# ersanjay16/Assignment--2-Group7-distributed-K-means

Measured on AMD Instinct MI355X. Metric: Lloyd iters/sec + points/sec, N=100M d=64 k=256, 1–8 GPUs; % of roofline, higher is better.
Workload: dtype f32; 1 GPU; c3: N=100000000 d=64 k=256; N=100000000, d=64, k=256, compute_sse=False, parallelism=dp1 (rows sharded, one RCCL all-reduce of k*(d+1) f64 per step)

## Files before the change

assignment--2-group7-distributed-k-means_amd/csrc/km_internal.h:

```cpp
#pragma once
#include <hip/hip_ext.h>
#include <hip/hip_runtime.h>
#include <stdint.h>

#include "../../include/kmeans_amd.h"

namespace km {

struct LaunchTiming {
  hipEvent_t start = nullptr, stop = nullptr;
};
extern thread_local LaunchTiming g_timing;
#define KM_TIMED_LAUNCH(KERNEL, GRID, BLOCK, LDS, STREAM, ...)                                               \
  do {                                                                                                     \
    if (::km::g_timing.start) {                                                                            \
      hipExtLaunchKernelGGL(KERNEL, GRID, BLOCK, LDS, STREAM, ::km::g_timing.start, ::km::g_timing.stop, 0, \
                            __VA_ARGS__);                                                                  \
      ::km::g_timing = ::km::LaunchTiming{};                                                               \
    } else {                                                                                               \
      hipLaunchKernelGGL(KERNEL, GRID, BLOCK, LDS, STREAM, __VA_ARGS__);                                    \
    }                                                                                                      \
  } while (0)

struct QEntry {
// ... 55 lines not shown
  int kp;
  uint32_t* qout = nullptr;
  int rev = 0;
};
hipError_t launch_assign_small(const float* X, const Geometry& g, const float* C32, const double* C64,
                               const float* cmax, int32_t* labels, double* stats, int fuse_stats, int want_sse,
                               int n_cu, const int* gate, hipStream_t s, const SmallTail& tail);
bool small_path_ok(const Geometry& g);
hipError_t launch_assign_mfma(const float* X, const Geometry& g, const _Float16* Chi, const _Float16* Clo,
                              const float* cn2s, const float* cmax, const float* xabs, const float* cabs,
                              int32_t* labels, QEntry* queue, uint32_t* qcount, int n_cu, QLayout* ql,
                              const int* gate, hipStream_t s, uint32_t* cand = nullptr, uint32_t* cand_ctr = nullptr,
                              uint32_t cand_cap = 0, int one = 0,
                              const float* C32 = nullptr, uint2* chg = nullptr, uint32_t* chg_cnt = nullptr);
int cand_rec_words();
size_t queue_capacity(int64_t n, int n_cu);
size_t qcount_words(int n_cu);
bool mfma_path_ok(const Geometry& g);
hipError_t launch_resolve(const float* X, const Geometry& g, const double* C64, const double* C64T,
                          const QEntry* queue, const uint32_t* qcount, const QLayout& ql, int32_t* labels,
                          double* stats, int n_cu, const int* gate, hipStream_t s, double* sse = nullptr,
                          const uint32_t* cand = nullptr, uint32_t cand_cap = 0, int delta = 0,
                          const float* sse_c32 = nullptr, uint2* chg = nullptr, const uint32_t* chg_cnt = nullptr,
                          const float* C32 = nullptr, const float* cmax = nullptr);
bool fused_path_ok(const Geometry& g);
#ifdef KM_DIAG
#endif
int diag_env(const char* name, int dflt);
enum { KM_SCREEN_X3 = 0, KM_SCREEN_X3_REFINE = 1, KM_SCREEN_FAST1 = 2, KM_SCREEN_FAST2 = 3 };
bool fast_path_ok(const Geometry& g);
hipError_t launch_fused(const float* X, const float* xnorm, const Geometry& g, const _Float16* Chi,
                        const _Float16* Clo, uint4* ChiF, uint4* CloF, const float* cn2s, const float* bnd,
                        const float* xabs, const float* cabs, int32_t* labels, QEntry* queue, uint32_t* qcount,
                        double* stats, int with_stats, int mode, int n_cu, QLayout* ql, const int* gate,
                        hipStream_t s, const float* C32, const float* cmax, float* bal, const double* C64P,
                        double* sse);
hipError_t launch_bound_consts(const float* cmax, const float* xabs, const float* cabs, const Geometry& g, float* bnd,
                               const int* gate, hipStream_t s);
bool fused16_ok(const Geometry& g);
hipError_t launch_row_norm(const float* X, const Geometry& g, float* xnorm, hipStream_t s);
bool stats_needs_sort(const Geometry& g, int extra);
void stats_ranges(const Geometry& g, int* fr_out, int* kr_out, int extra);
size_t sorted_stats_words(int64_t n, int k);
hipError_t launch_stats(const float* X, const Geometry& g, const int32_t* labels, const double* w, double* stats,
                        int n_cu, const int* gate, hipStream_t s, const double* C64, int c64s, const float* C32);
hipError_t launch_stats_sorted(const float* X, const Geometry& g, const int32_t* labels, const double* w,
                               double* stats, uint32_t* scratch, const double* C64P, int n_cu, const int* gate,
// ... 14 lines not shown
hipError_t launch_repair_pick(int* gate, const int64_t* counts, const Geometry& g, int64_t total,
                              double neg_log_delta, uint64_t seed, int32_t* empty, int32_t* pcounts, int64_t* picks,
                              int64_t* samples, int cp, const int64_t* sizes, const int64_t* bases, int nparts,
                              const float* X, int64_t row0, DevStatus* st, double* rows, int32_t* pending,
                              hipStream_t s);
hipError_t launch_repair_apply(int* gate, const Geometry& g, const int32_t* empty, const double* C_old,
                               double* C_new, DevStatus* st, double tol, const double* rows, const int32_t* pending,
                               hipStream_t s);
hipError_t launch_bernoulli(const uint64_t* seeds, const int64_t* sizes, const int64_t* bases, int nparts,
                            double fraction, int64_t* out, int cp, int32_t* counts, hipStream_t s);
bool s1_ok(const Geometry& g);
size_t s1_table_entries(const Geometry& g);
hipError_t launch_s1_color(const float* C32, const Geometry& g, int32_t* perm, const int* gate, hipStream_t s);
hipError_t launch_s1_prep(const double* C64, const float* C32, const Geometry& g, const int32_t* perm,
                          const float* cmax, const float* xabs, const float* cabs, float* cft, float* cn2o,
                          uint4* img, float* cst, const int* gate, hipStream_t s);
struct S1GateBufs;
hipError_t launch_s1(const float* X, const float* xnorm, const Geometry& g, const uint4* img, const float* cn2o,
                     const float* cft, const int32_t* perm, const float* cst, int32_t* labels,
                     QEntry* queue, uint32_t* qcount, uint2* chg, uint32_t* chg_cnt, int delta, int n_cu,
                     QLayout* ql, const int* gate, hipStream_t s, int rev = 0, double* sse = nullptr,
                     const S1GateBufs* gt = nullptr, int gdense = 0);
struct S1GateBufs {
  float* marg;
  uint2* wl;
  uint32_t* wl_cnt;
  double* cref;
  double* acc;
  float* accud;
};
bool s1_gate_ok(const Geometry& g);
hipError_t launch_s1_gate(const Geometry& g, const double* C64, const int32_t* labels, const S1GateBufs& b, int init,
                          const int32_t* init_dev, int n_cu, const int* gate, hipStream_t s);
size_t s1_chg_entries(const Geometry& g, int n_cu);
size_t s1_wave_slots(int n_cu);
bool s1_delta_ok(const Geometry& g, int n_cu);
hipError_t launch_s1_delta(const float* X, const Geometry& g, const uint2* chg, const uint32_t* chg_cnt,
                           double* stats, int n_cu, const int* gate, hipStream_t s, const uint32_t* qcount = nullptr);
hipError_t launch_chg_delta(const float* X, const Geometry& g, const uint2* chg, const uint32_t* chg_cnt, int nw,
                            uint32_t seg, double* stats, int n_cu, const int* gate, hipStream_t s,
                            const uint32_t* qcount = nullptr);
hipError_t launch_s1_apply(double* stats, double* full, int64_t len, int mode, const int* gate, hipStream_t s);
hipError_t launch_gen_blobs(float* X, const Geometry& g, int64_t row_offset, int32_t n_centers, float box,
                            float stddev, uint64_t seed, hipStream_t s);

__host__ __device__ inline uint64_t splitmix64(uint64_t z) {
  z += 0x9E3779B97F4A7C15ull;
// ... 18 lines not shown
```

assignment--2-group7-distributed-k-means_amd/csrc/km_kernels.hip:

```cpp
#include "km_exact.h"
#include "km_internal.h"

#include <float.h>
#include <algorithm>
#include <stdio.h>
#include <stdlib.h>

#ifndef KM_NARROW_WAVES
#define KM_NARROW_WAVES 16
#endif
#ifndef KM_WIDE_WAVES
#define KM_WIDE_WAVES 12
#endif
#ifndef KM_RERANK_PCT
#define KM_RERANK_PCT 100
#endif

namespace km {

thread_local LaunchTiming g_timing;

typedef float f32x16 __attribute__((ext_vector_type(16)));
typedef float f32x4 __attribute__((ext_vector_type(4)));

// ... 2836 lines not shown
      pre[b0 + i] = run;
      run += qcount[2 * (b0 + i) + which];
    }
  if (t == nt - 1) {
    uint32_t tot = 0;
    for (uint32_t i = 0; i < nt / 64; ++i) tot += wsum[i];
    pre[nseg] = tot;
  }
  __syncthreads();
}

__device__ __forceinline__ uint32_t find_segment(const uint32_t* __restrict__ pre, uint32_t nseg, uint32_t g) {
  uint32_t lo = 0, hi = nseg;
  while (hi - lo > 1) {
    const uint32_t mid = (lo + hi) >> 1;
    if (pre[mid] <= g)
      lo = mid;
    else
      hi = mid;
  }
  return lo;
}

template <bool WIDE, bool PF = false>
__global__ __launch_bounds__(WIDE ? 512 : 1024) void k_rerank2(const float* __restrict__ X, int dp, int d, int k,
                                                  const double* __restrict__ C64, const QEntry* __restrict__ queue,
                                                  const uint32_t* __restrict__ qcount, QLayout ql,
                                                  int32_t* __restrict__ labels, double* __restrict__ stats,
                                                  int tab_kp, double* __restrict__ sse, const int* __restrict__ gate,
                                                  const uint32_t* __restrict__ cand, uint32_t cand_cap, int delta,
                                                  const float* __restrict__ sse_c32, uint2* __restrict__ chg,
                                                  const uint32_t* __restrict__ chg_cnt,
                                                  const float* __restrict__ C32, const float* __restrict__ cmax) {
  if (*gate) return;
  extern __shared__ __attribute__((aligned(16))) char smem[];
  const float cmv = PF ? *cmax : 0.0f;
  double* tab = reinterpret_cast<double*>(smem);
  uint32_t* pre = reinterpret_cast<uint32_t*>(smem + (stats && tab_kp ? (size_t)(d + 1) * tab_kp * 8 : 0));
  uint32_t* pre1 = pre + ql.nwaves + 1;
  if (stats && tab_kp)
    for (int i = threadIdx.x; i < (d + 1) * tab_kp; i += blockDim.x) tab[i] = 0.0;
  block_prefix(qcount, 0, ql.nwaves, pre);
  if (stats && !delta) block_prefix(qcount, 1, ql.nwaves, pre1);
  const uint32_t total = pre[ql.nwaves];
  const int u = threadIdx.x & 7;
  const uint32_t ng = (gridDim.x * blockDim.x) >> 3;
  double ss_acc = 0.0;
  for (uint32_t g = (blockIdx.x * blockDim.x + threadIdx.x) >> 3; g < total + ((ng - total % ng) % ng);
       g += ng) {
    const bool have = g < total;
    QEntry q{0, 0, 0, 0};
    size_t cpos = 0;
    if (have) {
      const uint32_t sg = find_segment(pre, ql.nwaves, g);
      q = queue[(size_t)sg * ql.seg + (g - pre[sg])];
      if (delta) cpos = (size_t)sg * ql.seg + chg_cnt[sg] + (g - pre[sg]);
// ... 91 lines not shown
      mnorm = ua ? va : mnorm;
      bi = ua ? a : bi;
      const bool ub = bb != a && np_better(vb, mnorm, true);
      mnorm = ub ? vb : mnorm;
      bi = ub ? bb : bi;
    }
    lab = bi < 0 ? 0 : bi;
    if (!have) continue;
    double rsq_bad = 0.0;
    if (!ok && u == 0) {
      double best = 0.0;
      for (int j = 0; j < k; ++j) {
        const double* __restrict__ c = C64 + (size_t)j * d;
        const double v = np_norm_d<WIDE ? 5 : 2>([&](int f) { return np_sq(c[f], x[f]); }, d);
        const bool u = np_better(v, best, j > 0);
        best = u ? v : best;
        lab = u ? j : lab;
      }
      rsq_bad = best;
    }
    if (!ok) lab = __shfl(lab, (int)(threadIdx.x & 63) & ~7);
    const int old = delta ? (int)min((uint32_t)labels[q.row], (uint32_t)(k - 1)) : -1;
    if (u == 0) labels[q.row] = lab;
    if (sse && sse_c32) {
      double r = 0.0;
      for (int f = u; f < d; f += 8) {
        const double e = (double)x[f] - (double)sse_c32[(size_t)lab * dp + f];
        r = fma(e, e, r);
      }
      ss_acc += r;
    } else if (sse && u == 0) {
      const double mn = ok ? mnorm : rsq_bad;
      ss_acc += mn * mn;
    }
    if (delta) {
      if (u == 0) chg[cpos] = make_uint2(q.row, ((uint32_t)old << 16) | (uint32_t)lab);
    } else if (stats) {
      for (int f = u; f < d; f += 8) {
        if (tab_kp)
          atomicAdd(tab + (size_t)f * tab_kp + lab, (double)x[f]);
        else
          atomicAdd(stats + (size_t)lab * (d + 1) + f, (double)x[f]);
      }
      if (u == 0) {
        if (tab_kp)
          atomicAdd(tab + (size_t)d * tab_kp + lab, 1.0);
// ... 19 lines not shown
      if (u == 0) {
        if (tab_kp)
          atomicAdd(tab + (size_t)d * tab_kp + lab, 1.0);
        else
          atomicAdd(stats + (size_t)lab * (d + 1) + d, 1.0);
      }
    }
  }
  if (stats && tab_kp) {
    __syncthreads();
    for (int i = threadIdx.x; i < (d + 1) * tab_kp; i += blockDim.x) {
      const int j = i / (d + 1);
      const int f = i - j * (d + 1);
      const double v = tab[(size_t)f * tab_kp + j];
      if (v != 0.0 && j < k) atomicAdd(stats + (size_t)j * (d + 1) + f, v);
    }
  }
  if (sse) {
    ss_acc = wave_sum(ss_acc);
    if ((threadIdx.x & 63) == 0 && ss_acc != 0.0) atomicAdd(sse, ss_acc);
  }
}

template <int G, bool WIDE, bool PF = false>
__global__ __launch_bounds__(512) void k_fullscan(const float* __restrict__ X, int dp, int d, int k,
                                                   const double* __restrict__ C64T, const QEntry* __restrict__ queue,
                                                   const uint32_t* __restrict__ qcount, QLayout ql,
                                                   int32_t* __restrict__ labels, int ch,
                                                   double* __restrict__ stats, int use_chain, int pair_chain,
                                                   double* __restrict__ sse, const int* __restrict__ gate, int delta,
                                                   const float* __restrict__ sse_c32, uint2* __restrict__ chg,
                                                   const uint32_t* __restrict__ chg_cnt,
                                                   const float* __restrict__ C32, const float* __restrict__ cmax,
                                                   const double* __restrict__ C64r) {
  if (*gate) return;
  extern __shared__ __attribute__((aligned(16))) char smem[];
  double* sCT = reinterpret_cast<double*>(smem);
  float* xs_all = reinterpret_cast<float*>(smem + (size_t)d * ch * 8);
  uint32_t* pre = reinterpret_cast<uint32_t*>(smem + (size_t)d * ch * 8 + (size_t)8 * G * d * 4);
  uint32_t* kept_all = pre + ((ql.nwaves + 1u + 3u) & ~3u);
  const float cmv = PF ? *cmax : 0.0f;
  block_prefix(qcount, 1, ql.nwaves, pre);
  const uint32_t total = pre[ql.nwaves];
  const int lane = threadIdx.x & 63;
  const int wave = threadIdx.x >> 6;
  float* xs = xs_all + (size_t)wave * G * d;
  const uint32_t per_batch = 8u * G;
  double ss_acc = 0.0;
  for (uint32_t b0 = blockIdx.x * per_batch; b0 < total; b0 += gridDim.x * per_batch) {
    uint32_t rows[G];
    bool have[G];
    int chain[G];
    QEntry qe[G];
    size_t cpos[G];
#pragma unroll
    for (int g = 0; g < G; ++g) {
      const uint32_t e = b0 + (uint32_t)(wave * G + g);
// ... 23 lines not shown
#pragma unroll
      for (int g = 0; g < G; ++g)
        for (int f = 256 + lane; f < d; f += 64) xs[g * d + f] = X[(size_t)rows[g] * dp + f];
    auto finish = [&](int g, double bv, int bi) {
#pragma unroll
      for (int o = 32; o >= 1; o >>= 1) {
        const double ob = __shfl_xor(bv, o);
        const int oj = __shfl_xor(bi, o);
        bool take = false;
        if (oj >= 0) {
          if (bi < 0) {
            take = true;
          } else {
            const bool on = ob != ob, mn = bv != bv;
            take = (on && !mn) || (on == mn && (on ? oj < bi : (ob < bv || (ob == bv && oj < bi))));
          }
        }
        bv = take ? ob : bv;
        bi = take ? oj : bi;
      }
      const int lab = bi < 0 ? 0 : bi;
      const int old = delta ? (int)min((uint32_t)labels[rows[g]], (uint32_t)(k - 1)) : -1;
      if (lane == 0) labels[rows[g]] = lab;
      if (sse && sse_c32) {
        for (int f = lane; f < d; f += 64) {
          const double e = (double)xs[g * d + f] - (double)sse_c32[(size_t)lab * dp + f];
          ss_acc = fma(e, e, ss_acc);
        }
      } else if (sse && lane == 0 && bi >= 0) {
        ss_acc += bv * bv;
      }
      if (delta) {
        if (lane == 0) chg[cpos[g]] = make_uint2(rows[g], ((uint32_t)old << 16) | (uint32_t)lab);
      } else if (stats) {
        for (int f = lane; f < d; f += 64) atomicAdd(stats + (size_t)lab * (d + 1) + f, (double)xs[g * d + f]);
        if (lane == 0) atomicAdd(stats + (size_t)lab * (d + 1) + d, 1.0);
      }
    };
    if (k <= 256 && pair_chain) {
      static_assert(G % 2 == 0, "entry pairs");
#pragma unroll
      for (int p = 0; p < G; p += 2) {
        const bool a0 = have[p] && chain[p] >= 0, a1 = have[p + 1] && chain[p + 1] >= 0;
        if (!a0 && !a1) continue;
        const int e = lane >> 5;
        const int j = (e ? chain[p + 1] : chain[p]) + 8 * (lane & 31);
// ... 190 lines not shown
          const bool ua = have[g] && np_better(va, best[g], bj[g] >= 0);
          const bool ub = have[g + 1] && np_better(vb, best[g + 1], bj[g + 1] >= 0);
          best[g] = ua ? va : best[g];
          bj[g] = ua ? c0 + lane : bj[g];
          best[g + 1] = ub ? vb : best[g + 1];
          bj[g + 1] = ub ? c0 + lane : bj[g + 1];
        }
      }
    }
#pragma unroll
    for (int g = 0; g < G; ++g)
      if (have[g]) finish(g, best[g], bj[g]);
  }
  if (sse) {
    ss_acc = wave_sum(ss_acc);
    if (lane == 0 && ss_acc != 0.0) atomicAdd(sse, ss_acc);
  }
}

hipError_t launch_resolve(const float* X, const Geometry& g, const double* C64, const double* C64T,
                          const QEntry* queue, const uint32_t* qcount, const QLayout& ql, int32_t* labels,
                          double* stats, int n_cu, const int* gate, hipStream_t s, double* sse,
                          const uint32_t* cand, uint32_t cand_cap, int delta, const float* sse_c32, uint2* chg,
                          const uint32_t* chg_cnt, const float* C32, const float* cmax) {
  if (g.n == 0 || ql.nwaves == 0) return hipSuccess;
  if (delta && (!chg || !chg_cnt || g.k > 65535)) return hipErrorInvalidValue;
  if (delta) stats = nullptr;
  constexpr size_t LDS_MAX = 160 * 1024;
  const size_t pre_bytes = ((size_t)ql.nwaves + 1) * 4;
  if (pre_bytes > LDS_MAX / 4) return hipErrorInvalidValue;
  if (g.d > WIDE_MAX_DP) return hipErrorInvalidValue;
  static const int fs_g = diag_env("KM_FS_G", 0);
  const int G = fs_g == 4 ? 4 : (fs_g == 2 ? 2 : (g.k > 256 ? 4 : 2));
  const int ch = g.d <= 128 ? 64 : (g.d <= 256 ? 32 : 0);
  static const int fs_pf = diag_env("KM_FS_PF", 1);
  const bool pf = fs_pf && ch > 0 && C32 != nullptr && cmax != nullptr && g.d % 2 == 0 &&
                  (g.dp == 32 || g.dp == 64 || g.dp == 128 || g.dp == 256) && (size_t)ch * g.dp / 4 <= 4 * 512;
  const size_t fs_lds = (size_t)g.d * ch * 8 + (size_t)8 * G * g.d * 4 +
                        (pf ? (((size_t)ql.nwaves + 4) & ~(size_t)3) * 4 + (size_t)8 * G * 64 * 4 : pre_bytes);
  if (fs_lds > LDS_MAX) return hipErrorInvalidValue;
  static const int use_chain = diag_env("KM_CHAIN", 1);
  static const int pair_chain = diag_env("KM_PAIR_CHAIN", 1);
  static const int fs_wg = diag_env("KM_FS_WG", 1);
  if (ch == 0)
    hipLaunchKernelGGL((k_fullscan<2, true>), dim3(n_cu * fs_wg), dim3(512), fs_lds, s, X, g.dp, g.d, g.k, C64T,
                       queue, qcount, ql, labels, ch, (double*)nullptr, use_chain, pair_chain, sse, gate, delta, sse_c32, chg,
                       chg_cnt, C32, cmax, C64);
  else if (G == 4 && pf)
    hipLaunchKernelGGL((k_fullscan<4, false, true>), dim3(n_cu * fs_wg), dim3(512), fs_lds, s, X, g.dp, g.d, g.k,
                       C64T, queue, qcount, ql, labels, ch, (double*)nullptr, use_chain, pair_chain, sse, gate, delta,
                       sse_c32, chg, chg_cnt, C32, cmax, C64);
  else if (G == 4)
    hipLaunchKernelGGL((k_fullscan<4, false>), dim3(n_cu * fs_wg), dim3(512), fs_lds, s, X, g.dp, g.d, g.k, C64T,
                       queue, qcount, ql, labels, ch, (double*)nullptr, use_chain, pair_chain, sse, gate, delta, sse_c32, chg,
                       chg_cnt, C32, cmax, C64);
  else if (pf)
    hipLaunchKernelGGL((k_fullscan<2, false, true>), dim3(n_cu * fs_wg), dim3(512), fs_lds, s, X, g.dp, g.d, g.k,
                       C64T, queue, qcount, ql, labels, ch, (double*)nullptr, use_chain, pair_chain, sse, gate, delta,
                       sse_c32, chg, chg_cnt, C32, cmax, C64);
  else
    hipLaunchKernelGGL((k_fullscan<2, false>), dim3(n_cu * fs_wg), dim3(512), fs_lds, s, X, g.dp, g.d, g.k, C64T,
                       queue, qcount, ql, labels, ch, (double*)nullptr, use_chain, pair_chain, sse, gate, delta, sse_c32, chg,
                       chg_cnt, C32, cmax, C64);
  hipError_t e = hipGetLastError();
  if (e != hipSuccess) return e;
  const size_t tab_bytes = (size_t)(g.d + 1) * g.kp * 8;
  const size_t pres = (stats ? 2 : 1) * pre_bytes;
  const int tab_kp = (stats && !delta && tab_bytes + pres <= LDS_MAX) ? g.kp : 0;
  static const int rpct = diag_env("KM_RERANK_PCT", KM_RERANK_PCT);
  const int rwg = std::max(1, n_cu * std::max(1, rpct) / 100);
  static const int rr_pf = diag_env("KM_RR_PF", 1);
  if (g.d > 256)
    hipLaunchKernelGGL(k_rerank2<true>, dim3(rwg), dim3(512), (tab_kp ? tab_bytes : 0) + pres, s, X, g.dp, g.d,
                       g.k, C64, queue, qcount, ql, labels, stats, tab_kp, sse, gate, cand, cand_cap, delta, sse_c32, chg,
                       chg_cnt, C32, cmax);
  else if (rr_pf && g.d <= 128 && C32 && cmax)
    hipLaunchKernelGGL((k_rerank2<false, true>), dim3(rwg), dim3(1024), (tab_kp ? tab_bytes : 0) + pres, s, X, g.dp,
                       g.d, g.k, C64, queue, qcount, ql, labels, stats, tab_kp, sse, gate, cand, cand_cap, delta, sse_c32,
                       chg, chg_cnt, C32, cmax);
  else
    hipLaunchKernelGGL(k_rerank2<false>, dim3(rwg), dim3(1024), (tab_kp ? tab_bytes : 0) + pres, s, X, g.dp, g.d,
                       g.k, C64, queue, qcount, ql, labels, stats, tab_kp, sse, gate, cand, cand_cap, delta, sse_c32, chg,
                       chg_cnt, C32, cmax);
  return hipGetLastError();
}

static constexpr int STATS_LDS = 156 * 1024;

template <bool SSE, bool W>
__global__ __launch_bounds__(1024) void k_stats(const float* __restrict__ X, int64_t n, int d, int dp, int k,
                                                const int32_t* __restrict__ labels, double* __restrict__ stats,
                                                int kr, int fr, int64_t rows_per_block, const double* __restrict__ C64,
                                                const float* __restrict__ C32, double* __restrict__ sse,
                                                const int* __restrict__ gate, const double* __restrict__ w,
                                                double* __restrict__ wsum, int c64s) {
  if (*gate) return;
  if constexpr (!SSE) sse = nullptr;
  extern __shared__ __attribute__((aligned(16))) char smem[];
  double* tab = reinterpret_cast<double*>(smem);
  const int RS = fr + (W ? 2 : 1);
  const int L = fr / 4;
  const int c0 = blockIdx.y * kr;
  const int c1 = min(k, c0 + kr);
  const int f0 = blockIdx.z * fr;
  const bool counts = blockIdx.z == 0;
  const int nent = (c1 - c0) * RS;
// ... 870 lines not shown
```

assignment--2-group7-distributed-k-means_amd/csrc/km_runtime.hip:

```cpp
#include <stdlib.h>
#include <string.h>

#include <algorithm>
#include <cmath>
#include <string>
#include <utility>
#include <vector>

#include "../../include/kmeans_amd.h"
#include "km_internal.h"

namespace {
thread_local std::string g_err;

int fail(int code, const std::string& msg) {
  g_err = msg;
  return code;
}

#define KM_HIP(call)                                                                               \
  do {                                                                                             \
    hipError_t e_ = (call);                                                                        \
    if (e_ != hipSuccess)                                                                          \
      return fail(KM_ERR_HIP, std::string(#call) + ": " + hipGetErrorString(e_) + " (" +           \
// ... 522 lines not shown
  c->bounds_valid = false;
  if (!use_s1(c, with_stats)) c->gate_init_dev = nullptr;
  if (with_stats) c->last_gated = false;
  if (with_stats && !c->stats_clean) KM_HIP(hipMemsetAsync(c->stats, 0, sizeof(double) * stats_len(c), c->stream));
  if (with_stats) c->stats_clean = false;
  if (c->path == 1) {
    ProfScope ps(c, KM_K_ASSIGN, true);
    KM_HIP(km::launch_assign_small(c->X, g, c->C32, c->C64_cur, c->cmax, c->labels, c->stats, with_stats ? 1 : 0,
                                   sse ? 1 : 0, c->n_cu, c->gate, c->stream, small_tail(c)));
    c->ql = km::QLayout{0, g.n > 0 ? 1u : 0u};
    return KM_OK;
  }
  if (with_stats) {
    c->stats_pending = 1;
    c->last_delta = false;
    c->sse_corr = false;
  }
  if (use_s1(c, with_stats)) {
    double* s1_sse = sse ? sse_slot : nullptr;
    const bool gated = with_stats && !s1_sse && c->fused && g.n > 0 && km::s1_gate_ok(g);
    bool gdense = false;
    if (gated) {
      if (!c->gt.marg) {
        KM_HIP(hipMalloc(&c->gt.marg, sizeof(float) * (size_t)g.n));
        KM_HIP(hipMalloc(&c->gt.wl, sizeof(uint2) * km::s1_chg_entries(g, c->n_cu)));
        KM_HIP(hipMalloc(&c->gt.wl_cnt, sizeof(uint32_t) * km::s1_wave_slots(c->n_cu)));
        KM_HIP(hipMalloc(&c->gt.cref, sizeof(double) * (size_t)g.k * g.d));
        KM_HIP(hipMemsetAsync(c->gt.cref, 0, sizeof(double) * (size_t)g.k * g.d, c->stream));
        KM_HIP(hipMalloc(&c->gt.acc, sizeof(double) * (size_t)g.k));
        KM_HIP(hipMalloc(&c->gt.accud, sizeof(float) * 2 * (size_t)g.k));
        KM_HIP(hipMemsetAsync(c->gt.acc, 0, sizeof(double) * (size_t)g.k, c->stream));
        KM_HIP(hipMemsetAsync(c->gt.accud, 0, sizeof(float) * 2 * (size_t)g.k, c->stream));
      }
      gdense = !bounds_were_valid;
      ProfScope ps(c, KM_K_PREP);
      KM_HIP(km::launch_s1_gate(g, c->C64_cur, c->labels, c->gt, gdense ? 2 : 0, c->gate_init_dev, c->n_cu, c->gate,
                                c->stream));
    }
    c->gate_init_dev = nullptr;
    {
      ProfScope ps(c, KM_K_ASSIGN, true);
      KM_HIP(km::launch_s1(c->X, c->xnorm, g, c->s1_img, c->s1_cn2o, c->s1_cft, c->s1_perm, c->s1_cst,
                           c->labels, c->queue, c->qcount, c->chg, c->chg_cnt, with_stats ? 1 : 0, c->n_cu,
                           &c->ql, c->gate, c->stream, gated ? 0 : next_sweep(c), s1_sse,
                           gated ? &c->gt : nullptr, gdense ? 1 : 0));
    }
    if (gated) {
      c->bounds_valid = true;
      c->last_gated = true;
      c->gated_nw = c->ql.nwaves;
      c->gated_dense = gdense;
    }
    {
      ProfScope ps(c, KM_K_RESOLVE);
      KM_HIP(km::launch_resolve(c->X, g, c->C64_cur, c->C64T, c->queue, c->qcount, c->ql, c->labels, nullptr,
                                c->n_cu, c->gate, c->stream, s1_sse, nullptr, 0, with_stats ? 1 : 0,
                                s1_sse ? c->C32 : nullptr, c->chg, c->chg_cnt, c->C32, c->cmax));
    }
    if (with_stats) {
      ProfScope ps(c, KM_K_STATS);
      KM_HIP(km::launch_s1_delta(c->X, g, c->chg, c->chg_cnt, c->stats, c->n_cu, c->gate, c->stream, c->qcount));
    }
    if (with_stats) {
      c->stats_pending = 2;
      c->last_delta = true;
      c->sse_corr = s1_sse != nullptr;
    }
    return KM_OK;
  }
  if (c->fused) {
    {
      const int rc = ensure_x3(c);
      if (rc != KM_OK) return rc;
    }
    {
      ProfScope ps(c, KM_K_ASSIGN, true);
      KM_HIP(km::launch_fused(c->X, c->xnorm, g, c->Chi, c->Clo, c->ChiF, c->CloF, c->cn2s, c->bnd, c->xabs, c->cabs,
                              c->labels, c->queue, c->qcount, c->stats, with_stats ? 1 : 0,
                              (with_stats || c->screen >= km::KM_SCREEN_FAST1) ? c->screen : km::KM_SCREEN_X3_REFINE,
                              c->n_cu, &c->ql, c->gate, c->stream, c->C32, c->cmax, c->bal, c->C64P,
// ... 1157 lines not shown
```

assignment--2-group7-distributed-k-means_amd/csrc/km_s1_gate.h:

```cpp
#pragma once
#include <math.h>
#include <stdint.h>

#if defined(__HIPCC__) || defined(__CUDACC__)
#define KM_S1G_FN __host__ __device__ inline
#else
#define KM_S1G_FN inline
#endif

namespace km {

constexpr float S1G_U = 5.9604644775390625e-08f;
constexpr float S1G_TINY = 1e-30f;

KM_S1G_FN float s1g_up(float v) { return fmaf(fabsf(v), 8.0f * S1G_U, v) + S1G_TINY; }
KM_S1G_FN float s1g_dn(float v) { return fmaf(fabsf(v), -8.0f * S1G_U, v) - S1G_TINY; }

KM_S1G_FN float s1g_sqrt(float v) {
#if defined(__HIP_DEVICE_COMPILE__)
  return __builtin_amdgcn_sqrtf(v);
#else
  return sqrtf(v);
#endif
}
// ... 54 lines not shown
  const float f = (float)acc;
  const float r = fmaf(f, 0x1p-23f, f) + S1G_TINY;
  return (r <= 3.0e38f) ? r : INFINITY;
}
KM_S1G_FN float s1g_acc_dn(double acc) {
  if (!(acc <= 3.0e38)) return 0.0f;
  const float f = (float)acc;
  const float r = fmaf(f, -0x1p-23f, f) - S1G_TINY;
  return r > 0.0f ? r : 0.0f;
}
KM_S1G_FN double s1g_acc_pass(double acc, float sl, float so, float top, bool reset, float* up, float* dn) {
  const bool wild = !(top <= 3.0e38f);
  const double a = (reset || wild) ? 0.0 : s1g_acc_add(acc, sl, so);
  *up = (wild && !reset) ? INFINITY : s1g_acc_up(a);
  *dn = s1g_acc_dn(a);
  return a;
}
KM_S1G_FN float s1g_base(float marg, float acc_dn) {
  const float b = s1g_dn(marg + acc_dn);
  return (fabsf(b) <= 3.0e38f) ? b : 0.0f;
}
KM_S1G_FN bool s1g_keep(float base, float acc_up) { return base > acc_up; }

KM_S1G_FN float s1g_xnorm(float xs) {
  float v = s1g_up(xs * (1.0f + 64.0f * S1G_U));
  v = !(v < 0x1p-96f) ? v : 0x1p-96f;
  return s1g_up(s1g_up(s1g_sqrt(v)));
}

}
```

assignment--2-group7-distributed-k-means_amd/csrc/km_screen1.hip:

```cpp
#include <float.h>

#include <type_traits>

#include "km_internal.h"
#include "km_s1_gate.h"
#include "km_s1_ring.h"

namespace km {

namespace {

typedef _Float16 f16x8 __attribute__((ext_vector_type(8)));
typedef float f32x4 __attribute__((ext_vector_type(4)));
typedef float f32x2 __attribute__((ext_vector_type(2)));
typedef _Float16 f16x2 __attribute__((ext_vector_type(2)));

constexpr float U24 = 5.9604644775390625e-08f;
constexpr float U16 = 4.8828125e-04f;
#ifndef KM_S1_LMAX
#define KM_S1_LMAX 8
#endif
constexpr int S1_LMAX = KM_S1_LMAX;
#ifndef KM_S1_NBUF
#define KM_S1_NBUF 0
// ... 28 lines not shown
  const int dp = 32 * ns2, kp = 32 * nb, nt = 32 << ceil_log2_c(nb);
  return (size_t)kp * dp * 2 + (table ? (size_t)nt * (dp + 4) * 4 : 0) + (size_t)kp * 4 + (size_t)nt * 4 +
         (s1_batched(ns2) ? (size_t)s1_waves(ns2, nb) * s1_ring(ns2, nb) * (dp * 4 + 16 + 128) : 0);
}
constexpr bool s1_table_global(int ns2, int nb) { return s1_lds_bytes(ns2, nb, true) > 160 * 1024; }
#ifndef KM_S1_GATE
#define KM_S1_GATE 1
#endif
constexpr size_t s1_gate_ring_lds(int ns2, int nb) { return (size_t)s1_waves(ns2, nb) * s1_ring(ns2, nb) * 4; }
constexpr size_t s1_gate_lds(int ns2, int nb) { return s1_gate_ring_lds(ns2, nb) + (size_t)32 * nb * 4; }
constexpr bool s1_gated_with(int ns2, int nb, size_t extra) {
  return KM_S1_GATE && s1_batched(ns2) && s1_tiles(ns2) == 1 && !s1_table_global(ns2, nb) &&
         s1_lds_bytes(ns2, nb, true) + extra <= 160 * 1024;
}
constexpr bool s1_gated(int ns2, int nb) { return s1_gated_with(ns2, nb, s1_gate_lds(ns2, nb)); }
constexpr bool s1_gated_kept(int ns2, int nb) {
  return s1_gated(ns2, nb) == s1_gated_with(ns2, nb, s1_gate_ring_lds(ns2, nb));
}
static_assert(s1_gated_kept(2, 2) && s1_gated_kept(2, 4) && s1_gated_kept(2, 6) && s1_gated_kept(2, 8) &&
                  s1_gated_kept(1, 2) && s1_gated_kept(1, 4) && s1_gated_kept(1, 6) && s1_gated_kept(1, 8) &&
                  s1_gated_kept(1, 12) && s1_gated_kept(1, 16),
              "the lower totals' LDS table must not cost a geometry its gate");
static_assert(!KM_S1_GATE || !KM_S1_W12 || s1_gated(2, 8), "the c3 geometry is gated");


__device__ __forceinline__ uint32_t f2u(float v) { return __float_as_uint(v); }
__device__ __forceinline__ float u2f(uint32_t v) { return __uint_as_float(v); }

__device__ __forceinline__ float min_raw(float a, float b) {
  float r;
  asm("v_min_f32 %0, %1, %2" : "=v"(r) : "v"(a), "v"(b));
  return r;
}
__device__ __forceinline__ float min3_raw(float a, float b, float c) {
  float r;
  asm("v_min3_f32 %0, %1, %2, %3" : "=v"(r) : "v"(a), "v"(b), "v"(c));
  return r;
}

__device__ __forceinline__ float quad_min(float v) {
  auto p = __builtin_amdgcn_permlane16_swap(f2u(v), f2u(v), false, false);
  v = min_raw(u2f(p[0]), u2f(p[1]));
  p = __builtin_amdgcn_permlane32_swap(f2u(v), f2u(v), false, false);
  return min_raw(u2f(p[0]), u2f(p[1]));
}
__device__ __forceinline__ float quad_sum(float v) {
// ... 135 lines not shown
  }
}

struct S1Args {
  const float* X;
  const float* xnorm;
  int64_t n;
  int k, d;
  uint32_t seg;
  const uint4* img;
  const float* cn2o;
  const float* cft;
  const int32_t* perm;
  const float* cst;
  int32_t* labels;
  QEntry* queue;
  uint32_t* qcount;
  uint2* chg;
  uint32_t* chg_cnt;
  double* sse;
  const int* gate;
  const uint2* wl;
  const uint32_t* wl_cnt;
  float* marg;
  const float* acc_dn;
};

template <int NS2, int NB, int MODE, bool REV = false, bool SSE = false, int GATED = 0>
__global__ __launch_bounds__(s1_waves(NS2, NB) * 64, s1_waves(NS2, NB) / 4) void k_s1(S1Args A) {
  if (*A.gate) return;
  constexpr int S1_WAVES = s1_waves(NS2, NB);
  constexpr int S1_RING = s1_ring(NS2, NB);
  static_assert(S1_RING == 12 || S1_RING == 16, "ring sizes covered by s1_ring_check");
  static_assert(16 <= 2 * S1_RING && S1_TILE_ROWS == 16, "a tile may complete at most two batches");
  static_assert(!GATED || (MODE == 1 && !REV && !SSE && s1_batched(NS2)), "the gated instance: delta mode, batched");
  constexpr bool LIST = GATED == 1;
  constexpr bool MARG = GATED != 0;
  constexpr int DP = 32 * NS2;
  constexpr int FQ = 8 * NS2;
  constexpr int KP = 32 * NB;
  constexpr int MB = ceil_log2_c(NB);
  constexpr int NT = 32 << MB;
  constexpr int CS = DP + 4;
  constexpr uint32_t SLOTM = (uint32_t)NT - 1u;
  constexpr uint32_t KMASK = ~SLOTM;
  constexpr float RHO = (float)SLOTM * 1.1920928955078125e-07f * 1.0001f;
  constexpr bool BATCH = s1_batched(NS2);
// ... 228 lines not shown
      {
        const float4* hp = sRh + ((wave * S1_RING + slot) * 4 + q) * 2;
        const float4 h0 = hp[0], h1 = hp[1];
        const float hv[8] = {h0.x, h0.y, h0.z, h0.w, h1.x, h1.y, h1.z, h1.w};
        float prev = u2f(mt.w);
#pragma unroll
        for (int r = 1; r < S1_LMAX; ++r) {
          if (__ballot(act && (uint32_t)r < cnt) == 0ull) break;
          float nl = FLT_MAX;
#pragma unroll
          for (int i = 0; i < 8; ++i) nl = min_raw(nl, hv[i] > prev ? hv[i] : FLT_MAX);
          prev = quad_min(nl);
          sl[r] = (uint32_t)r < cnt ? (f2u(prev) & SLOTM) : 0u;
        }
      }
      int32_t lab1 = 0, lab2 = 0;
      uint32_t kind = 2u, ws = 0u;
      float ubw = 0.0f, lbo = 0.0f;
      decide(act, cnt, sl, xv, lab1, lab2, kind, ws, ubw, lbo);
      emit(act, mt.x, kind, lab1, lab2, (int32_t)(mt.y & 0xFFFFu));
      resid(act && kind == 0u, ws, xv);
      if constexpr (MARG) {
        if (act && q == 0)
          A.marg[mt.x] = (kind == 0u && gscale)
                             ? s1g_base(s1g_margin(fminf(lbo, sRl[wave * S1_RING + slot]), ubw), sAd[lab1])
                             : 0.0f;
      }
    } else {
      (void)nb;
    }
  };

  auto tail = [&](uint32_t tile, const Buf& B, const float (&h)[2][4], float h2m) {
    uint32_t row;
    uint32_t lold = 0u;
    if constexpr (LIST) {
      row = wpick(wg0.x, wsub);
      lold = wpick(wg0.y, wsub);
    } else {
      row = tmap(tile) * 16u + (uint32_t)c16;
    }
    const bool valid = row < n;
    float hk[2][4];
#pragma unroll
    for (int cb = 0; cb < 2; ++cb)
#pragma unroll
      for (int i = 0; i < 4; ++i) hk[cb][i] = u2f(f2u(h[cb][i]) | qbits | ((uint32_t)(16 * cb + i) << MB));

    auto mn = [](float a, float b) { return __builtin_fminf(a, b); };
// ... 67 lines not shown
    const int32_t labm = sPerm[sm];
    const bool dec1 = ok && cnt == 1u && labm >= 0;
    int32_t old = 0;
    if constexpr (LIST)
      old = (int32_t)min(lold, (uint32_t)(A.k - 1));
    else if constexpr (MODE == 1)
      old = (int32_t)min((uint32_t)B.old, (uint32_t)(A.k - 1));
#if KM_S1_ABL == 2
    emit(valid, row, dec1 || needy ? 0u : 2u, labm, 0, old);
    return;
#endif
    float lbT = 0.0f;
    if constexpr (MARG) {
      const S1GRow gr = s1g_row(s, E, xq);
      float nl = h2m;
#pragma unroll
      for (int cb = 0; cb < 2; ++cb)
#pragma unroll
        for (int i = 0; i < 4; ++i) nl = min_raw(nl, hk[cb][i] > m ? hk[cb][i] : FLT_MAX);
      const float h2 = quad_min(nl);
      lbT = s1g_lb(T, RP, gr);
      if (valid && !needy && q == 0)
        A.marg[row] =
            (dec1 && gscale) ? s1g_base(s1g_margin(s1g_lb(h2, RP, gr), s1g_ub(m, RP, gr)), sAd[labm]) : 0.0f;
    }
    if constexpr (BATCH) {
      emit(valid && !needy, row, dec1 ? 0u : 2u, labm, 0, old);
      resid(dec1, sm, B.x);
      const uint64_t mrow = __ballot(needy && q == 0);
      if (mrow) {
        const uint32_t nn = (uint32_t)__popcll(mrow);
        const uint32_t rk = (uint32_t)__popcll(mrow & ((1ull << c16) - 1ull));
        const uint32_t space = (uint32_t)S1_RING - rc;
        const uint4 meta = make_uint4(row, (uint32_t)old | (cnt << 16), sm, f2u(la));
        auto stash = [&](uint32_t slot) {
          float4* xs = reinterpret_cast<float4*>(sRx + (wave * S1_RING + slot) * DP + FQ * q);
#pragma unroll
          for (int u = 0; u < FQ / 4; ++u) xs[u] = B.x[u];
          if (q == 0) sRm[wave * S1_RING + slot] = meta;
          float4* hp = sRh + ((wave * S1_RING + slot) * 4 + q) * 2;
          hp[0] = make_float4(hk[0][0], hk[0][1], hk[0][2], hk[0][3]);
          hp[1] = make_float4(hk[1][0], hk[1][1], hk[1][2], hk[1][3]);
          if constexpr (MARG)
            if (q == 0) sRl[wave * S1_RING + slot] = lbT;
        };
        constexpr bool EARLY0 = !SSE;
        if (EARLY0 && needy && rk < space) stash(rc + rk);
// ... 282 lines not shown
      m1 = fmaxf(m1, om1);
    }
    if (lane == 0) {
      stop[0] = m1;
      stop[1] = fmaxf(m2, 0.0f);
      stop[2] = __int_as_float(a1);
    }
  }
  __syncthreads();
  {
    const float top1 = stop[0], top2 = stop[1];
    const int atop = __float_as_int(stop[2]);
    for (int j = threadIdx.x; j < k; j += blockDim.x) {
      float up, dn;
      acc[j] = s1g_acc_pass(acc[j], sv[j], j == atop ? top2 : top1, top1, reset != 0, &up, &dn);
      accud[j] = up;
      accud[k + j] = dn;
    }
  }
}

struct S1GateArgs {
  const int32_t* labels;
  const float* marg;
  int64_t n;
  int k;
  uint32_t seg;
  const float* acc_up;
  uint2* wl;
  uint32_t* wl_cnt;
  int init;
  const int32_t* init_dev;
  const int* gate;
};

constexpr int S1G_UNITS = 2;
constexpr uint32_t S1G_TRIP = 256u * S1G_UNITS;

template <int WAVES>
__global__ __launch_bounds__(WAVES * 64) void k_s1_gate(S1GateArgs A) {
  if (*A.gate) return;
  __shared__ float sUp[1024];
  for (int i = threadIdx.x; i < A.k; i += WAVES * 64) sUp[i] = A.acc_up[i];
  __syncthreads();
  const int lane = threadIdx.x & 63, wave = threadIdx.x >> 6;
  const uint32_t gw = blockIdx.x * WAVES + wave;
  const uint64_t n = (uint64_t)A.n;
  const uint64_t r0 = (uint64_t)gw * A.seg, r1 = max(r0, min(n, r0 + A.seg));
  uint2* wl = A.wl + (size_t)gw * A.seg;
  const uint64_t below = (1ull << lane) - 1ull;
  const bool init = A.init != 0 || (A.init_dev && *A.init_dev != 0);
  const uint32_t km1 = (uint32_t)(A.k - 1);
  uint32_t cnt = 0;
  struct Trip {
    int4 lab[S1G_UNITS];
    float4 bs[S1G_UNITS];
  };
  auto fetch = [&](uint64_t base, Trip& T) {
#pragma unroll
    for (int u = 0; u < S1G_UNITS; ++u) {
      const uint64_t row = base + 256u * u + 4u * (uint32_t)lane;
      T.lab[u] = *reinterpret_cast<const int4*>(A.labels + row);
      T.bs[u] = init ? make_float4(0.0f, 0.0f, 0.0f, 0.0f) : *reinterpret_cast<const float4*>(A.marg + row);
    }
  };
  auto fetch_tail = [&](uint64_t base, Trip& T) {
#pragma unroll
    for (int u = 0; u < S1G_UNITS; ++u) {
      const uint64_t row = base + 256u * u + 4u * (uint32_t)lane;
      int32_t l[4];
      float b[4];
#pragma unroll
      for (int i = 0; i < 4; ++i) {
        const bool in = row + i < r1;
        l[i] = in ? A.labels[row + i] : 0;
        b[i] = (in && !init) ? A.marg[row + i] : 0.0f;
      }
      T.lab[u] = make_int4(l[0], l[1], l[2], l[3]);
      T.bs[u] = make_float4(b[0], b[1], b[2], b[3]);
    }
  };
  auto sift = [&](uint64_t base, const Trip& T) {
#pragma unroll
    for (int u = 0; u < S1G_UNITS; ++u) {
      const uint64_t row = base + 256u * u + 4u * (uint32_t)lane;
      auto clampk = [&](int32_t v) -> uint32_t { return (uint32_t)v < km1 ? (uint32_t)v : km1; };
      const uint32_t l[4] = {clampk(T.lab[u].x), clampk(T.lab[u].y), clampk(T.lab[u].z), clampk(T.lab[u].w)};
      const float b[4] = {T.bs[u].x, T.bs[u].y, T.bs[u].z, T.bs[u].w};
      bool ls[4];
      uint32_t c = 0;
#pragma unroll
      for (int i = 0; i < 4; ++i) {
        ls[i] = row + i < r1 && (init || !s1g_keep(b[i], sUp[l[i]]));
        c += ls[i] ? 1u : 0u;
      }
      const uint64_t b0 = __ballot((c & 1u) != 0u), b1 = __ballot((c & 2u) != 0u), b2 = __ballot((c & 4u) != 0u);
      if ((b0 | b1 | b2) == 0ull) continue;
      uint32_t pos = cnt + (uint32_t)__popcll(b0 & below) + 2u * (uint32_t)__popcll(b1 & below) +
                     4u * (uint32_t)__popcll(b2 & below);
#pragma unroll
      for (int i = 0; i < 4; ++i)
        if (ls[i]) wl[pos++] = make_uint2((uint32_t)(row + i), l[i]);
      cnt += (uint32_t)__popcll(b0) + 2u * (uint32_t)__popcll(b1) + 4u * (uint32_t)__popcll(b2);
    }
  };
  const uint64_t rfull = r0 + (r1 - r0) / S1G_TRIP * S1G_TRIP;
  uint64_t base = r0;
  if (base < rfull) {
    Trip ta, tb;
    fetch(base, ta);
    tb = ta;
// ... 361 lines not shown
```

Before: 1241 Lloyd it/s.

## Pack gate margin and label into one word to halve gate-kernel reads

The S1 gate margin buffer now stores a packed 32-bit word: the margin base float with its low 9 mantissa bits replaced by the label. The screening and resolve kernels (rerank, fullscan) write this packed word, so the gate kernel reads one stream instead of both labels and margins. The gate unroll factor also rises from 2 to 4 units. In exchange, margin precision drops slightly, the resolve kernels do extra scattered writes, and labels are limited to 512.

```diff
diff --git a/assignment--2-group7-distributed-k-means_amd/csrc/km_internal.h b/assignment--2-group7-distributed-k-means_amd/csrc/km_internal.h
--- a/assignment--2-group7-distributed-k-means_amd/csrc/km_internal.h
+++ b/assignment--2-group7-distributed-k-means_amd/csrc/km_internal.h
@@ -101,7 +101,7 @@
                           double* stats, int n_cu, const int* gate, hipStream_t s, double* sse = nullptr,
                           const uint32_t* cand = nullptr, uint32_t cand_cap = 0, int delta = 0,
                           const float* sse_c32 = nullptr, uint2* chg = nullptr, const uint32_t* chg_cnt = nullptr,
-                          const float* C32 = nullptr, const float* cmax = nullptr);
+                          const float* C32 = nullptr, const float* cmax = nullptr, uint32_t* gword = nullptr);
 bool fused_path_ok(const Geometry& g);
 #ifdef KM_DIAG
 #endif
@@ -162,7 +162,7 @@
                      QLayout* ql, const int* gate, hipStream_t s, int rev = 0, double* sse = nullptr,
                      const S1GateBufs* gt = nullptr, int gdense = 0);
 struct S1GateBufs {
-  float* marg;
+  uint32_t* marg;
   uint2* wl;
   uint32_t* wl_cnt;
   double* cref;
diff --git a/assignment--2-group7-distributed-k-means_amd/csrc/km_kernels.hip b/assignment--2-group7-distributed-k-means_amd/csrc/km_kernels.hip
--- a/assignment--2-group7-distributed-k-means_amd/csrc/km_kernels.hip
+++ b/assignment--2-group7-distributed-k-means_amd/csrc/km_kernels.hip
@@ -1,5 +1,6 @@
 #include "km_exact.h"
 #include "km_internal.h"
+#include "km_s1_gate.h"
 
 #include <float.h>
 #include <algorithm>
@@ -2882,7 +2883,9 @@
   return lo;
 }
 
-template <bool WIDE, bool PF = false>
+__device__ __forceinline__ uint32_t* gate_word_of(uint32_t* p) { return p; }
+
+template <bool WIDE, bool PF = false, typename... GW>
 __global__ __launch_bounds__(WIDE ? 512 : 1024) void k_rerank2(const float* __restrict__ X, int dp, int d, int k,
                                                   const double* __restrict__ C64, const QEntry* __restrict__ queue,
                                                   const uint32_t* __restrict__ qcount, QLayout ql,
@@ -2891,7 +2894,8 @@
                                                   const uint32_t* __restrict__ cand, uint32_t cand_cap, int delta,
                                                   const float* __restrict__ sse_c32, uint2* __restrict__ chg,
                                                   const uint32_t* __restrict__ chg_cnt,
-                                                  const float* __restrict__ C32, const float* __restrict__ cmax) {
+                                                  const float* __restrict__ C32, const float* __restrict__ cmax,
+                                                  GW... gword) {
   if (*gate) return;
   extern __shared__ __attribute__((aligned(16))) char smem[];
   const float cmv = PF ? *cmax : 0.0f;
@@ -3029,6 +3033,8 @@
     if (!ok) lab = __shfl(lab, (int)(threadIdx.x & 63) & ~7);
     const int old = delta ? (int)min((uint32_t)labels[q.row], (uint32_t)(k - 1)) : -1;
     if (u == 0) labels[q.row] = lab;
+    if constexpr (sizeof...(GW) != 0)
+      if (u == 0) gate_word_of(gword...)[q.row] = s1g_pack(0.0f, (uint32_t)lab);
     if (sse && sse_c32) {
       double r = 0.0;
       for (int f = u; f < d; f += 8) {
@@ -3094,7 +3100,7 @@
   }
 }
 
-template <int G, bool WIDE, bool PF = false>
+template <int G, bool WIDE, bool PF = false, typename... GW>
 __global__ __launch_bounds__(512) void k_fullscan(const float* __restrict__ X, int dp, int d, int k,
                                                    const double* __restrict__ C64T, const QEntry* __restrict__ queue,
                                                    const uint32_t* __restrict__ qcount, QLayout ql,
@@ -3104,7 +3110,7 @@
                                                    const float* __restrict__ sse_c32, uint2* __restrict__ chg,
                                                    const uint32_t* __restrict__ chg_cnt,
                                                    const float* __restrict__ C32, const float* __restrict__ cmax,
-                                                   const double* __restrict__ C64r) {
+                                                   const double* __restrict__ C64r, GW... gword) {
   if (*gate) return;
   extern __shared__ __attribute__((aligned(16))) char smem[];
   double* sCT = reinterpret_cast<double*>(smem);
@@ -3174,6 +3180,8 @@
       const int lab = bi < 0 ? 0 : bi;
       const int old = delta ? (int)min((uint32_t)labels[rows[g]], (uint32_t)(k - 1)) : -1;
       if (lane == 0) labels[rows[g]] = lab;
+      if constexpr (sizeof...(GW) != 0)
+        if (lane == 0) gate_word_of(gword...)[rows[g]] = s1g_pack(0.0f, (uint32_t)lab);
       if (sse && sse_c32) {
         for (int f = lane; f < d; f += 64) {
           const double e = (double)xs[g * d + f] - (double)sse_c32[(size_t)lab * dp + f];
@@ -3410,9 +3418,10 @@
                           const QEntry* queue, const uint32_t* qcount, const QLayout& ql, int32_t* labels,
                           double* stats, int n_cu, const int* gate, hipStream_t s, double* sse,
                           const uint32_t* cand, uint32_t cand_cap, int delta, const float* sse_c32, uint2* chg,
-                          const uint32_t* chg_cnt, const float* C32, const float* cmax) {
+                          const uint32_t* chg_cnt, const float* C32, const float* cmax, uint32_t* gword) {
   if (g.n == 0 || ql.nwaves == 0) return hipSuccess;
   if (delta && (!chg || !chg_cnt || g.k > 65535)) return hipErrorInvalidValue;
+  if (gword && (!delta || g.kp > (1 << S1G_LBITS))) return hipErrorInvalidValue;
   if (delta) stats = nullptr;
   constexpr size_t LDS_MAX = 160 * 1024;
   const size_t pre_bytes = ((size_t)ql.nwaves + 1) * 4;
@@ -3430,26 +3439,30 @@
   static const int use_chain = diag_env("KM_CHAIN", 1);
   static const int pair_chain = diag_env("KM_PAIR_CHAIN", 1);
   static const int fs_wg = diag_env("KM_FS_WG", 1);
-  if (ch == 0)
-    hipLaunchKernelGGL((k_fullscan<2, true>), dim3(n_cu * fs_wg), dim3(512), fs_lds, s, X, g.dp, g.d, g.k, C64T,
-                       queue, qcount, ql, labels, ch, (double*)nullptr, use_chain, pair_chain, sse, gate, delta, sse_c32, chg,
-                       chg_cnt, C32, cmax, C64);
+#define KM_FS_LAUNCH(KERNEL_, ...)                                                                              \
+  hipLaunchKernelGGL(KERNEL_, dim3(n_cu * fs_wg), dim3(512), fs_lds, s, X, g.dp, g.d, g.k, C64T, queue, qcount, ql, \
+                     labels, ch, (double*)nullptr, use_chain, pair_chain, sse, gate, delta, sse_c32, chg, chg_cnt,  \
+                     C32, cmax, C64, ##__VA_ARGS__)
+  if (gword && ch == 0) return hipErrorInvalidValue;
+  if (gword && G == 4 && pf)
+    KM_FS_LAUNCH((k_fullscan<4, false, true, uint32_t*>), gword);
+  else if (gword && G == 4)
+    KM_FS_LAUNCH((k_fullscan<4, false, false, uint32_t*>), gword);
+  else if (gword && pf)
+    KM_FS_LAUNCH((k_fullscan<2, false, true, uint32_t*>), gword);
+  else if (gword)
+    KM_FS_LAUNCH((k_fullscan<2, false, false, uint32_t*>), gword);
+  else if (ch == 0)
+    KM_FS_LAUNCH((k_fullscan<2, true>));
   else if (G == 4 && pf)
-    hipLaunchKernelGGL((k_fullscan<4, false, true>), dim3(n_cu * fs_wg), dim3(512), fs_lds, s, X, g.dp, g.d, g.k,
-                       C64T, queue, qcount, ql, labels, ch, (double*)nullptr, use_chain, pair_chain, sse, gate, delta,
-                       sse_c32, chg, chg_cnt, C32, cmax, C64);
+    KM_FS_LAUNCH((k_fullscan<4, false, true>));
   else if (G == 4)
-    hipLaunchKernelGGL((k_fullscan<4, false>), dim3(n_cu * fs_wg), dim3(512), fs_lds, s, X, g.dp, g.d, g.k, C64T,
-                       queue, qcount, ql, labels, ch, (double*)nullptr, use_chain, pair_chain, sse, gate, delta, sse_c32, chg,
-                       chg_cnt, C32, cmax, C64);
+    KM_FS_LAUNCH((k_fullscan<4, false>));
   else if (pf)
-    hipLaunchKernelGGL((k_fullscan<2, false, true>), dim3(n_cu * fs_wg), dim3(512), fs_lds, s, X, g.dp, g.d, g.k,
-                       C64T, queue, qcount, ql, labels, ch, (double*)nullptr, use_chain, pair_chain, sse, gate, delta,
-                       sse_c32, chg, chg_cnt, C32, cmax, C64);
+    KM_FS_LAUNCH((k_fullscan<2, false, true>));
   else
-    hipLaunchKernelGGL((k_fullscan<2, false>), dim3(n_cu * fs_wg), dim3(512), fs_lds, s, X, g.dp, g.d, g.k, C64T,
-                       queue, qcount, ql, labels, ch, (double*)nullptr, use_chain, pair_chain, sse, gate, delta, sse_c32, chg,
-                       chg_cnt, C32, cmax, C64);
+    KM_FS_LAUNCH((k_fullscan<2, false>));
+#undef KM_FS_LAUNCH
   hipError_t e = hipGetLastError();
   if (e != hipSuccess) return e;
   const size_t tab_bytes = (size_t)(g.d + 1) * g.kp * 8;
@@ -3458,18 +3471,22 @@
   static const int rpct = diag_env("KM_RERANK_PCT", KM_RERANK_PCT);
   const int rwg = std::max(1, n_cu * std::max(1, rpct) / 100);
   static const int rr_pf = diag_env("KM_RR_PF", 1);
-  if (g.d > 256)
-    hipLaunchKernelGGL(k_rerank2<true>, dim3(rwg), dim3(512), (tab_kp ? tab_bytes : 0) + pres, s, X, g.dp, g.d,
-                       g.k, C64, queue, qcount, ql, labels, stats, tab_kp, sse, gate, cand, cand_cap, delta, sse_c32, chg,
-                       chg_cnt, C32, cmax);
+#define KM_RR_LAUNCH(KERNEL_, THREADS_, ...)                                                                     \
+  hipLaunchKernelGGL(KERNEL_, dim3(rwg), dim3(THREADS_), (tab_kp ? tab_bytes : 0) + pres, s, X, g.dp, g.d, g.k, C64, \
+                     queue, qcount, ql, labels, stats, tab_kp, sse, gate, cand, cand_cap, delta, sse_c32, chg,       \
+                     chg_cnt, C32, cmax, ##__VA_ARGS__)
+  if (gword && g.d > 128) return hipErrorInvalidValue;
+  if (gword && rr_pf && C32 && cmax)
+    KM_RR_LAUNCH((k_rerank2<false, true, uint32_t*>), 1024, gword);
+  else if (gword)
+    KM_RR_LAUNCH((k_rerank2<false, false, uint32_t*>), 1024, gword);
+  else if (g.d > 256)
+    KM_RR_LAUNCH((k_rerank2<true>), 512);
   else if (rr_pf && g.d <= 128 && C32 && cmax)
-    hipLaunchKernelGGL((k_rerank2<false, true>), dim3(rwg), dim3(1024), (tab_kp ? tab_bytes : 0) + pres, s, X, g.dp,
-                       g.d, g.k, C64, queue, qcount, ql, labels, stats, tab_kp, sse, gate, cand, cand_cap, delta, sse_c32,
-                       chg, chg_cnt, C32, cmax);
+    KM_RR_LAUNCH((k_rerank2<false, true>), 1024);
   else
-    hipLaunchKernelGGL(k_rerank2<false>, dim3(rwg), dim3(1024), (tab_kp ? tab_bytes : 0) + pres, s, X, g.dp, g.d,
-                       g.k, C64, queue, qcount, ql, labels, stats, tab_kp, sse, gate, cand, cand_cap, delta, sse_c32, chg,
-                       chg_cnt, C32, cmax);
+    KM_RR_LAUNCH((k_rerank2<false>), 1024);
+#undef KM_RR_LAUNCH
   return hipGetLastError();
 }
 
diff --git a/assignment--2-group7-distributed-k-means_amd/csrc/km_runtime.hip b/assignment--2-group7-distributed-k-means_amd/csrc/km_runtime.hip
--- a/assignment--2-group7-distributed-k-means_amd/csrc/km_runtime.hip
+++ b/assignment--2-group7-distributed-k-means_amd/csrc/km_runtime.hip
@@ -568,7 +568,7 @@
     bool gdense = false;
     if (gated) {
       if (!c->gt.marg) {
-        KM_HIP(hipMalloc(&c->gt.marg, sizeof(float) * (size_t)g.n));
+        KM_HIP(hipMalloc(&c->gt.marg, sizeof(uint32_t) * (size_t)g.n));
         KM_HIP(hipMalloc(&c->gt.wl, sizeof(uint2) * km::s1_chg_entries(g, c->n_cu)));
         KM_HIP(hipMalloc(&c->gt.wl_cnt, sizeof(uint32_t) * km::s1_wave_slots(c->n_cu)));
         KM_HIP(hipMalloc(&c->gt.cref, sizeof(double) * (size_t)g.k * g.d));
@@ -601,7 +601,8 @@
       ProfScope ps(c, KM_K_RESOLVE);
       KM_HIP(km::launch_resolve(c->X, g, c->C64_cur, c->C64T, c->queue, c->qcount, c->ql, c->labels, nullptr,
                                 c->n_cu, c->gate, c->stream, s1_sse, nullptr, 0, with_stats ? 1 : 0,
-                                s1_sse ? c->C32 : nullptr, c->chg, c->chg_cnt, c->C32, c->cmax));
+                                s1_sse ? c->C32 : nullptr, c->chg, c->chg_cnt, c->C32, c->cmax,
+                                gated ? c->gt.marg : nullptr));
     }
     if (with_stats) {
       ProfScope ps(c, KM_K_STATS);
diff --git a/assignment--2-group7-distributed-k-means_amd/csrc/km_s1_gate.h b/assignment--2-group7-distributed-k-means_amd/csrc/km_s1_gate.h
--- a/assignment--2-group7-distributed-k-means_amd/csrc/km_s1_gate.h
+++ b/assignment--2-group7-distributed-k-means_amd/csrc/km_s1_gate.h
@@ -100,6 +100,33 @@
 }
 KM_S1G_FN bool s1g_keep(float base, float acc_up) { return base > acc_up; }
 
+constexpr int S1G_LBITS = 9;
+constexpr uint32_t S1G_LMASK = (1u << S1G_LBITS) - 1u;
+
+KM_S1G_FN uint32_t s1g_bits(float v) {
+#if defined(__HIP_DEVICE_COMPILE__)
+  return __float_as_uint(v);
+#else
+  uint32_t u;
+  __builtin_memcpy(&u, &v, 4);
+  return u;
+#endif
+}
+KM_S1G_FN float s1g_float(uint32_t u) {
+#if defined(__HIP_DEVICE_COMPILE__)
+  return __uint_as_float(u);
+#else
+  float v;
+  __builtin_memcpy(&v, &u, 4);
+  return v;
+#endif
+}
+KM_S1G_FN uint32_t s1g_pack(float base, uint32_t label) {
+  return ((base > 0.0f) ? (s1g_bits(base) & ~S1G_LMASK) : 0u) | (label & S1G_LMASK);
+}
+KM_S1G_FN float s1g_word_base(uint32_t w) { return s1g_float(w & ~S1G_LMASK); }
+KM_S1G_FN uint32_t s1g_word_label(uint32_t w) { return w & S1G_LMASK; }
+
 KM_S1G_FN float s1g_xnorm(float xs) {
   float v = s1g_up(xs * (1.0f + 64.0f * S1G_U));
   v = !(v < 0x1p-96f) ? v : 0x1p-96f;
diff --git a/assignment--2-group7-distributed-k-means_amd/csrc/km_screen1.hip b/assignment--2-group7-distributed-k-means_amd/csrc/km_screen1.hip
--- a/assignment--2-group7-distributed-k-means_amd/csrc/km_screen1.hip
+++ b/assignment--2-group7-distributed-k-means_amd/csrc/km_screen1.hip
@@ -74,6 +74,13 @@
                   s1_gated_kept(1, 12) && s1_gated_kept(1, 16),
               "the lower totals' LDS table must not cost a geometry its gate");
 static_assert(!KM_S1_GATE || !KM_S1_W12 || s1_gated(2, 8), "the c3 geometry is gated");
+constexpr bool s1_gate_label_fits(int ns2, int nb) { return !s1_gated(ns2, nb) || 32 * nb <= (1 << S1G_LBITS); }
+static_assert(s1_gate_label_fits(2, 2) && s1_gate_label_fits(2, 4) && s1_gate_label_fits(2, 6) &&
+                  s1_gate_label_fits(2, 8) && s1_gate_label_fits(1, 2) && s1_gate_label_fits(1, 4) &&
+                  s1_gate_label_fits(1, 6) && s1_gate_label_fits(1, 8) && s1_gate_label_fits(1, 12) &&
+                  s1_gate_label_fits(1, 16) && s1_gate_label_fits(1, 32) && s1_gate_label_fits(2, 16) &&
+                  s1_gate_label_fits(4, 2) && s1_gate_label_fits(4, 4),
+              "a gated geometry's labels must fit the gate word");
 
 
 __device__ __forceinline__ uint32_t f2u(float v) { return __float_as_uint(v); }
@@ -255,7 +262,7 @@
   const int* gate;
   const uint2* wl;
   const uint32_t* wl_cnt;
-  float* marg;
+  uint32_t* marg;
   const float* acc_dn;
 };
 
@@ -530,9 +537,12 @@
       resid(act && kind == 0u, ws, xv);
       if constexpr (MARG) {
         if (act && q == 0)
-          A.marg[mt.x] = (kind == 0u && gscale)
-                             ? s1g_base(s1g_margin(fminf(lbo, sRl[wave * S1_RING + slot]), ubw), sAd[lab1])
-                             : 0.0f;
+          A.marg[mt.x] =
+              kind == 0u
+                  ? s1g_pack(gscale ? s1g_base(s1g_margin(fminf(lbo, sRl[wave * S1_RING + slot]), ubw), sAd[lab1])
+                                    : 0.0f,
+                             (uint32_t)lab1)
+                  : s1g_pack(0.0f, mt.y & 0xFFFFu);
       }
     } else {
       (void)nb;
@@ -646,7 +656,9 @@
       lbT = s1g_lb(T, RP, gr);
       if (valid && !needy && q == 0)
         A.marg[row] =
-            (dec1 && gscale) ? s1g_base(s1g_margin(s1g_lb(h2, RP, gr), s1g_ub(m, RP, gr)), sAd[labm]) : 0.0f;
+            dec1 ? s1g_pack(gscale ? s1g_base(s1g_margin(s1g_lb(h2, RP, gr), s1g_ub(m, RP, gr)), sAd[labm]) : 0.0f,
+                            (uint32_t)labm)
+                 : s1g_pack(0.0f, (uint32_t)old);
     }
     if constexpr (BATCH) {
       emit(valid && !needy, row, dec1 ? 0u : 2u, labm, 0, old);
@@ -975,7 +987,7 @@
 
 struct S1GateArgs {
   const int32_t* labels;
-  const float* marg;
+  const uint32_t* marg;
   int64_t n;
   int k;
   uint32_t seg;
@@ -987,7 +999,7 @@
   const int* gate;
 };
 
-constexpr int S1G_UNITS = 2;
+constexpr int S1G_UNITS = 4;
 constexpr uint32_t S1G_TRIP = 256u * S1G_UNITS;
 
 template <int WAVES>
@@ -1005,41 +1017,40 @@
   const bool init = A.init != 0 || (A.init_dev && *A.init_dev != 0);
   const uint32_t km1 = (uint32_t)(A.k - 1);
   uint32_t cnt = 0;
+  const uint32_t* src = init ? reinterpret_cast<const uint32_t*>(A.labels) : A.marg;
   struct Trip {
-    int4 lab[S1G_UNITS];
-    float4 bs[S1G_UNITS];
+    uint4 w[S1G_UNITS];
   };
   auto fetch = [&](uint64_t base, Trip& T) {
 #pragma unroll
     for (int u = 0; u < S1G_UNITS; ++u) {
       const uint64_t row = base + 256u * u + 4u * (uint32_t)lane;
-      T.lab[u] = *reinterpret_cast<const int4*>(A.labels + row);
-      T.bs[u] = init ? make_float4(0.0f, 0.0f, 0.0f, 0.0f) : *reinterpret_cast<const float4*>(A.marg + row);
+      T.w[u] = *reinterpret_cast<const uint4*>(src + row);
     }
   };
   auto fetch_tail = [&](uint64_t base, Trip& T) {
 #pragma unroll
     for (int u = 0; u < S1G_UNITS; ++u) {
       const uint64_t row = base + 256u * u + 4u * (uint32_t)lane;
-      int32_t l[4];
-      float b[4];
-#pragma unroll
-      for (int i = 0; i < 4; ++i) {
-        const bool in = row + i < r1;
-        l[i] = in ? A.labels[row + i] : 0;
-        b[i] = (in && !init) ? A.marg[row + i] : 0.0f;
-      }
-      T.lab[u] = make_int4(l[0], l[1], l[2], l[3]);
-      T.bs[u] = make_float4(b[0], b[1], b[2], b[3]);
+      uint32_t w[4];
+#pragma unroll
+      for (int i = 0; i < 4; ++i) w[i] = row + i < r1 ? src[row + i] : 0u;
+      T.w[u] = make_uint4(w[0], w[1], w[2], w[3]);
     }
   };
   auto sift = [&](uint64_t base, const Trip& T) {
 #pragma unroll
     for (int u = 0; u < S1G_UNITS; ++u) {
       const uint64_t row = base + 256u * u + 4u * (uint32_t)lane;
-      auto clampk = [&](int32_t v) -> uint32_t { return (uint32_t)v < km1 ? (uint32_t)v : km1; };
-      const uint32_t l[4] = {clampk(T.lab[u].x), clampk(T.lab[u].y), clampk(T.lab[u].z), clampk(T.lab[u].w)};
-      const float b[4] = {T.bs[u].x, T.bs[u].y, T.bs[u].z, T.bs[u].w};
+      const uint32_t w[4] = {T.w[u].x, T.w[u].y, T.w[u].z, T.w[u].w};
+      auto clampk = [&](uint32_t v) -> uint32_t { return v < km1 ? v : km1; };
+      uint32_t l[4];
+      float b[4];
+#pragma unroll
+      for (int i = 0; i < 4; ++i) {
+        l[i] = clampk(init ? w[i] : s1g_word_label(w[i]));
+        b[i] = init ? 0.0f : s1g_word_base(w[i]);
+      }
       bool ls[4];
       uint32_t c = 0;
 #pragma unroll
```

Result: faster. 1316 Lloyd it/s, median of 6 (+6.0%).
